# AaronZ345/StyleSinger

Hardware: AMD Instinct MI355X
Metric: mel-frames/sec (end-to-end infer incl. vocoder) (higher is better)
Workload: dtype f32; 1 GPU; c2: batch=8x8.0s utterances per GPU (T=1500 frames, Tp=28, Tr=1500), 100 mel + 2x100 f0 diffusion steps + HiFi-GAN-NSF, exact fp32 MFMA; global_batch=8, frames_per_utterance=1500, parallelism=dp1, diffusion_loops=hipGraph replay, hipgraph_captures=6, frame_bucket=64, mfma_precision=fp32, step_overlap=3 HIP streams: consecutive batches run concurrently

## Files before the change

include/stylesinger_hip.h:

```cpp
#ifndef STYLESINGER_HIP_H
#define STYLESINGER_HIP_H

#include <stdint.h>

#ifdef __cplusplus
extern "C" {
#endif

#define SS_ABI_VERSION 20
#define SS_MAX_TAPS 16
#define SS_MAX_LAYERS 32

const char* ss_last_error(void);
int ss_abi_version(void);
int ss_device_info(int dev, int* n_cu, char* arch, int arch_len);
int ss_struct_sizes(int64_t* out, int n);
int ss_set_tuning(const char* key, int value);
int ss_get_tuning(const char* key);
int ss_set_clock_probe(void* dev_u64x2);
int ss_set_q4_guard(void* dev_u32x2);
int ss_debug_null_launch(int grid, int block, void* stream);

enum {
  SS_EPI_STORE = 0,
// ... 14 lines not shown
  int32_t tap_off[SS_MAX_TAPS];
  const int32_t* lens;
  int32_t B, T;
  const float* a_bias;
  float a_scale;
  float a_lrelu;
  const float* W;
  int32_t N;
  int32_t Np;
  int32_t Kp;
  int32_t epi;
  const float* bias;
  float pre_scale;
  int32_t act;
  float act_slope;
  const float* E;
  int32_t lde;
  int64_t e_batch_stride;
  int32_t gate_mode;
  const float* R;
  int32_t ldr;
  int64_t r_batch_stride;
  float post_scale;
  int32_t accumulate;
  int32_t mask_rows;
  float* C;
  int32_t ldc;
  int64_t c_batch_stride;
  float* C2;
  int32_t ldc2;
  int64_t c2_batch_stride;
  int32_t Nh;
  float ddpm_recip, ddpm_recipm1, ddpm_c1, ddpm_c2, ddpm_sigma;
  const float* noise;
  uint64_t seed;
  const uint64_t* seed_dev;
  uint32_t step;
  int32_t tile;
  int32_t group_size;
  int64_t w_group_stride, bias_group_stride, a_bias_group_stride;
  int32_t mfma_bf16;
  int32_t ddpm_x0_pred;
  int32_t e_tiled;
  int32_t reserved2_;
} ss_conv_gemm_args;

int ss_conv_gemm(const ss_conv_gemm_args* args, void* stream);

int ss_gemm16_res(const ss_conv_gemm_args* args, int mt, void* stream);
int ss_gemm16_pick(int B, int T, int N);
int ss_gemm16_store(const ss_conv_gemm_args* args, int mt, void* stream);
int ss_gemm16_store_splitk(const ss_conv_gemm_args* args, int mt, int ksplit, float* partials, void* stream);
int ss_gemm16_ksplit_pick(int B, int T, int N, int K);

int ss_gemm16_resw(const ss_conv_gemm_args* args, const float* W16, int mt, void* stream);
int ss_pack_gemm16_weights(const float* src, float* dst, int Np, int Kp, void* stream);
int ss_wino43_gate16w(const ss_conv_gemm_args* args, const float* W16, int dilation, int mt, void* stream);
int ss_pack_gate16_weights(const float* src, float* dst, int Np, int Kp, void* stream);
int ss_wino43_gate16x(const ss_conv_gemm_args* args, const void* Wx, int dilation, int mt, void* stream);
int ss_split3_weights(const float* src, void* dst, int Np, int Kp, void* stream);
int ss_gemm16x_store(const ss_conv_gemm_args* args, const void* Wx, int mt, void* stream);
int ss_split3_gemm16_weights(const float* src, void* dst, int Np, int Kp, void* stream);
int64_t ss_split3_gemm16_elems(int Np, int Kp);
int ss_wino43_conv(const ss_conv_gemm_args* args, int k, int dilation, void* stream);
int ss_wino43_conv_ok(int C, int k, int dilation);
int ss_wino43_conv_ok4(int Cin, int Cout, int k, int dilation);
int ss_wino44_conv(const ss_conv_gemm_args* args, int k, int dilation, void* stream);
int ss_wino44_conv_ok(int C, int k, int dilation);
int ss_wino_gate(const ss_conv_gemm_args* args, int dilation, void* stream);
int ss_wino_weight_transform(const float* src, float* dst, int Cout, int Cin, void* stream);
int ss_wino43_gate(const ss_conv_gemm_args* args, int dilation, void* stream);
int ss_wino43_gate16(const ss_conv_gemm_args* args, int dilation, int mt, void* stream);
int ss_gate16_tile_addend(const float* E, int lde, int64_t e_batch_stride, float* E16, int B, int T, int Np, int dilation, int mt, void* stream);
int64_t ss_gate16_tiled_floats(int B, int T, int Np, int dilation, int mt);
int ss_wino43_gate16_pick(int B, int T, int Np, int dilation);
int ss_wino43_weight_transform(const float* src, float* dst, int Cout, int Cin, void* stream);

enum {
  SS_HEPI_STORE = 0,
  SS_HEPI_GATE = 1,
  SS_HEPI_RESX = 2
};
typedef struct ss_gemm_bf16_args {
  const uint16_t* A;
  int64_t a_batch_stride;
  int32_t lda;
  int32_t K;
  int32_t ntaps;
  int32_t tap_off[4];
  const int32_t* lens;
  int32_t B, T;
  const uint16_t* W;
  int64_t w_group_stride;
  int32_t N, Np;
  int32_t epi;
  int32_t act;
  const float* bias;
  int64_t bias_group_stride;
  const float* E;
  int32_t lde;
  int32_t gate_mode;
  int64_t e_batch_stride;
  float* X;
  int64_t x_batch_stride;
  int32_t ldx;
  float post_scale;
// ... 350 lines not shown
```

stylesinger_amd/csrc/common.h:

```cpp
#pragma once
#include <hip/hip_runtime.h>
#include <stdint.h>
#include <stdio.h>
#include <string.h>
#include <math.h>

#define SS_OK 0
#define SS_ERR_ARG (-1)
#define SS_ERR_HIP (-2)
#define SS_ERR_UNSUPPORTED (-3)

void ss_set_error(const char* fmt, ...);

#define SS_CHECK_ARG(cond, ...)            \
  do {                                     \
    if (!(cond)) {                         \
      ss_set_error(__VA_ARGS__);           \
      return SS_ERR_ARG;                   \
    }                                      \
  } while (0)

#define SS_CHECK_LAUNCH(name)                                                   \
  do {                                                                          \
    hipError_t e__ = hipGetLastError();                                         \
    if (e__ != hipSuccess) {                                                    \
      ss_set_error("%s: launch failed: %s", name, hipGetErrorString(e__));      \
      return SS_ERR_HIP;                                                        \
    }                                                                           \
  } while (0)

#define SS_PROPAGATE(expr)        \
  do {                            \
    int rc__ = (expr);            \
    if (rc__ != SS_OK) return rc__; \
  } while (0)

static inline int ss_cdiv(long a, long b) { return (int)((a + b - 1) / b); }

struct SsTuning { unsigned long long* clock_probe; int gate16; int gate256; int gate16_ks; int voc_wino_max_mb; int mel_tail; int gate128; int q4_force;
                  int layer512; int layer512_tail; int skip_dense; };
extern SsTuning g_ss_tuning;
extern unsigned int* g_ss_q4_guard;
struct ss_gemm_bf16_args;
int ss_q4_guard_launch(const ss_gemm_bf16_args* a, int which, void* stream);
int ss_n_cu();
struct ss_conv_gemm_args;
int ss_gemm16_store_partials(const ss_conv_gemm_args* args, int mt, int ksplit, float* partials, void* stream);

__device__ __forceinline__ int ss_uniform_len(const int* lens, int b, int T) {
  if (!lens) return T;
  const auto* p = reinterpret_cast<const __attribute__((address_space(4))) int*>(reinterpret_cast<uintptr_t>(lens));
  const int n = p[__builtin_amdgcn_readfirstlane(b)];
  return n < T ? (n < 0 ? 0 : n) : T;
}
__device__ __forceinline__ float ss_sigmoid(float x) { return 1.0f / (1.0f + expf(-x)); }
__device__ __forceinline__ float ss_sigmoid_fast(float x) { return __builtin_amdgcn_rcpf(1.0f + __expf(-x)); }
__device__ __forceinline__ float ss_tanh_fast(float x) { return 2.0f * __builtin_amdgcn_rcpf(1.0f + __expf(-2.0f * x)) - 1.0f; }
__device__ __forceinline__ float ss_gelu(float x) { return 0.5f * x * (1.0f + erff(x * 0.70710678118654752440f)); }
__device__ __forceinline__ float ss_mish(float x) {
  float sp = (x > 20.0f) ? x : log1pf(expf(x));
  return x * tanhf(sp);
}
__device__ __forceinline__ float ss_lrelu(float x, float slope) { return x >= 0.0f ? x : x * slope; }
__device__ __forceinline__ float ss_lrelu_max(float x, float sx) {
  float o;
  asm("v_max_f32 %0, %1, %2" : "=v"(o) : "v"(x), "v"(sx));
  return o;
}

enum SsAct { SS_ACT_NONE = 0, SS_ACT_RELU = 1, SS_ACT_GELU = 2, SS_ACT_MISH = 3, SS_ACT_TANH = 4, SS_ACT_LRELU = 5 };

__device__ __forceinline__ float ss_apply_act(float v, int act, float slope) {
  switch (act) {
    case SS_ACT_RELU: return fmaxf(v, 0.0f);
    case SS_ACT_GELU: return ss_gelu(v);
    case SS_ACT_MISH: return ss_mish(v);
    case SS_ACT_TANH: return tanhf(v);
    case SS_ACT_LRELU: return ss_lrelu(v, slope);
    default: return v;
  }
}

struct SsPhilox {
  uint32_t k0, k1;
  __device__ __forceinline__ SsPhilox(uint64_t seed) : k0((uint32_t)seed), k1((uint32_t)(seed >> 32)) {}
  __device__ __forceinline__ void round(uint32_t (&c)[4], uint32_t ka, uint32_t kb) const {
    const uint32_t M0 = 0xD2511F53u, M1 = 0xCD9E8D57u;
    uint32_t hi0 = __umulhi(M0, c[0]), lo0 = M0 * c[0];
    uint32_t hi1 = __umulhi(M1, c[2]), lo1 = M1 * c[2];
    uint32_t n0 = hi1 ^ c[1] ^ ka, n1 = lo1, n2 = hi0 ^ c[3] ^ kb, n3 = lo0;
    c[0] = n0; c[1] = n1; c[2] = n2; c[3] = n3;
  }
  __device__ __forceinline__ void gen(uint32_t c0, uint32_t c1, uint32_t c2, uint32_t c3, uint32_t (&out)[4]) const {
    uint32_t c[4] = {c0, c1, c2, c3};
    uint32_t ka = k0, kb = k1;
#pragma unroll
    for (int i = 0; i < 10; ++i) {
      round(c, ka, kb);
      ka += 0x9E3779B9u;
      kb += 0xBB67AE85u;
// ... 52 lines not shown
```

stylesinger_amd/csrc/diffusion.hip:

```cpp
#include "common.h"
#include <stdlib.h>
#include <cmath>
#include <vector>
#include "../../include/stylesinger_hip.h"

namespace {

inline int64_t align_up(int64_t x, int64_t a) { return (x + a - 1) / a * a; }
inline int round_up32(int x) { return (x + 31) / 32 * 32; }
constexpr int MTR = 2;

enum StackKind {
  STACK_FP32,
  STACK_PAIR16,
  STACK_FUSED16,
};
enum GateEntry { GATE_CONV, GATE_WINO23, GATE_WINO43, GATE_WINO43_16, GATE_WINO43_16W, GATE_WINO43_16X };
enum ProjEntry { PROJ_CONV, PROJ_RES16, PROJ_RES16W };
enum SkipEntry { SKIP_CONV, SKIP_STORE16, SKIP_SPLITK, SKIP_X3 };
struct LayerForm {
  int d;
  GateEntry gate;
  int mt;
  int64_t e16_floats;
// ... 179 lines not shown
  a.lda = ld;
  a.a_batch_stride = (int64_t)T * ld;
}
template <class Args, class P> inline void set_c(Args& a, P* p, int ld, int T) {
  a.C = p;
  a.ldc = ld;
  a.c_batch_stride = (int64_t)T * ld;
}
template <class Args> inline void set_taps3(Args& a, int d) {
  a.ntaps = 3;
  a.tap_off[0] = -d;
  a.tap_off[1] = 0;
  a.tap_off[2] = d;
}
inline void set_groups(ss_conv_gemm_args& a, const ss_wavenet* net, int B, int64_t gs_w, int64_t gs_bias, int64_t gs_a_bias = 0) {
  if (net->n_groups <= 1) return;
  a.group_size = B / net->n_groups;
  a.w_group_stride = gs_w;
  a.bias_group_stride = gs_bias;
  a.a_bias_group_stride = gs_a_bias;
}

int precompute_cond(const ss_wavenet* net, const StackForm& sf, const float* cond, const int32_t* lens, int B, int T, const WsLayout& w, hipStream_t stream) {
  const int NE = net->L * 2 * net->C;
  if (sf.cond16) {
    SS_PROPAGATE(ss_to_bf16(cond, nullptr, w.condh, B, T, net->cond_dim, net->cond_dim, net->cond_dim, nullptr, 0, 0, stream));
    ss_gemm_bf16_args h = base_args_h(net, B, T, lens);
    set_a(h, w.condh, net->cond_dim, T);
    h.K = net->cond_dim;
    h.W = net->w_cond_h;
    h.w_group_stride = net->gs_w_cond_h;
    h.N = NE;
    h.Np = NE;
    h.epi = SS_HEPI_STORE;
    h.bias = net->b_cond;
    h.bias_group_stride = net->gs_b_cond;
    set_c(h, w.E, NE, T);
    h.mask_rows = 0;
    return ss_gemm_bf16(&h, stream);
  }
  ss_conv_gemm_args a = base_args(B, T, lens);
  set_a(a, cond, net->cond_dim, T);
  a.Cin = net->cond_dim;
  a.W = net->w_cond;
  a.N = NE;
  a.Np = NE;
  a.Kp = round_up32(net->cond_dim);
  a.epi = SS_EPI_STORE;
  a.bias = net->b_cond;
  set_c(a, w.E, NE, T);
  a.mask_rows = 0;
  a.mfma_bf16 = sf.outer_bf16;
  set_groups(a, net, B, net->gs_w_cond, net->gs_b_cond);
  SS_PROPAGATE(ss_conv_gemm(&a, stream));
  for (int l = 0; l < net->L; ++l) {
    const float* El = w.E + (int64_t)l * 2 * net->C;
    if (w.E512)
      SS_PROPAGATE(ss_layer512_tile_addend(El, NE, (int64_t)T * NE, w.E512 + (int64_t)l * w.e512_layer, B, T, stream));
    if (w.E512h)
      SS_PROPAGATE(ss_layer512_tile_addend_f16(El, NE, (int64_t)T * NE, w.E512h + (int64_t)l * w.e512h_layer, sf.n_esets, w.e512h_set, B, T, stream));
    if (w.E16[l])
      SS_PROPAGATE(ss_gate16_tile_addend(El, NE, (int64_t)T * NE, w.E16[l], B, T, 2 * net->C, sf.layer[l].d, sf.layer[l].mt, stream));
  }
  return SS_OK;
}

int skip_gemm_f32(const ss_wavenet* net, const StackForm& sf, const int32_t* lens, int B, int T, const WsLayout& w, hipStream_t stream, bool leave_partials) {
  const int C = net->C, L = net->L;
  ss_conv_gemm_args k = base_args(B, T, lens);
  set_a(k, w.GA, L * C, T);
  k.Cin = L * C;
  k.W = net->w_skipall;
  k.N = C;
  k.Np = round_up32(C);
  k.Kp = L * C;
  k.epi = SS_EPI_STORE;
  k.bias = net->b_skipall;
  set_c(k, sf.skip_folded ? w.G : w.S, C, T);
  if (sf.skip_folded) k.act = SS_ACT_RELU;
  k.tile = SS_TILE_64x64;
  k.mfma_bf16 = sf.conv_bf16;
  set_groups(k, net, B, net->gs_w_skipall, net->gs_b_skipall);
  switch (sf.skip) {
    case SKIP_X3:
      k.w_group_stride = net->gs_w_skipall_x3;
      return ss_gemm16x_store(&k, net->w_skipall_x3, sf.mt16, stream);
    case SKIP_SPLITK:
      return leave_partials && sf.partials_ok ? ss_gemm16_store_partials(&k, 4, sf.ksplit, w.KP, stream) : ss_gemm16_store_splitk(&k, 4, sf.ksplit, w.KP, stream);
    case SKIP_STORE16: return ss_gemm16_store(&k, sf.mt16, stream);
    default: return ss_conv_gemm(&k, stream);
  }
}

int run_stack_f32(const ss_wavenet* net, const StackForm& sf, int step, const int32_t* lens, int B, int T, const WsLayout& w, hipStream_t stream, bool leave_partials) {
  const int C = net->C, L = net->L;
  const int NE = L * 2 * C;
  const int ldg = sf.defer ? L * C : C;
  for (int l = 0; l < L; ++l) {
    const LayerForm& y = sf.layer[l];
    ss_conv_gemm_args a = base_args(B, T, lens);
    set_a(a, w.X, C, T);
    a.Cin = C;
    set_taps3(a, y.d);
    a.a_bias = net->dstep + ((int64_t)step * L + l) * C;
    a.W = net->w_dil[l];
    a.N = C;
    a.Np = 2 * C;
// ... 453 lines not shown
  const float fa = (f0_a[i] + 1.0f) / 2.0f * (10.0f - 6.0f) + 6.0f;
  const float fb = (f0_b[i] + 1.0f) / 2.0f * (10.0f - 6.0f) + 6.0f;
  const float f = fb / 2.0f + fa / 2.0f;
  const float u = ub / 2.0f + ua / 2.0f;
  pitch_pred[(int64_t)i * 2 + 0] = f;
  pitch_pred[(int64_t)i * 2 + 1] = u;
  float hz = exp2f(f);
  if (u > 0.0f) hz = 0.0f;
  if (mel2ph[i] == 0) hz = 0.0f;
  f0_denorm[i] = hz;
  coarse[i] = f0_to_coarse(hz);
}

__global__ void pitch_given_kernel(const float* __restrict__ f0_log2, const float* __restrict__ uv, const int64_t* __restrict__ mel2ph,
                                   float* __restrict__ pitch_pred, float* __restrict__ f0_denorm, int64_t* __restrict__ coarse, int n) {
  const int i = blockIdx.x * blockDim.x + threadIdx.x;
  if (i >= n) return;
  const float f = f0_log2[i] / 2.0f + f0_log2[i] / 2.0f;
  const float u = uv[i] / 2.0f + uv[i] / 2.0f;
  pitch_pred[(int64_t)i * 2 + 0] = f;
  pitch_pred[(int64_t)i * 2 + 1] = u;
  float hz = exp2f(f);
  if (u > 0.0f) hz = 0.0f;
  if (mel2ph[i] == 0) hz = 0.0f;
  f0_denorm[i] = hz;
  coarse[i] = f0_to_coarse(hz);
}

inline int grid_for(int64_t n) {
  int64_t g = (n + 255) / 256;
  return (int)(g < 1 ? 1 : (g > 8192 ? 8192 : g));
}

}

extern "C" int64_t ss_wavenet_workspace_bytes(const ss_wavenet* net, int B, int T) {
  if (!net || B <= 0 || T <= 0) return -1;
  return ws_layout(net, resolve_form(net, B, T), B, T, nullptr).bytes;
}

static int mel_input_proj(const ss_wavenet* net, const float* x_in, const int32_t* lens, int B, int T, const WsLayout& w, hipStream_t stream) {
  const int C = net->C, M = net->in_dim;
  ss_conv_gemm_args a = base_args(B, T, lens);
  set_a(a, x_in, M, T);
  a.Cin = M;
  a.W = net->w_in;
  a.N = C;
  a.Np = round_up32(C);
  a.Kp = round_up32(M);
  a.epi = SS_EPI_STORE;
  a.bias = net->b_in;
  a.act = SS_ACT_RELU;
  set_c(a, w.X, C, T);
  return ss_conv_gemm(&a, stream);
}

__global__ __launch_bounds__(256) void mel_tail_kernel(const SkipSrc src, const float* __restrict__ Wf, const float* __restrict__ bf,
                                                       float* __restrict__ x, const float* __restrict__ noise, uint64_t seed,
                                                       const uint64_t* __restrict__ seed_dev, uint32_t step, float recip, float recipm1, float c1,
                                                       float c2, float sigma, const float* __restrict__ Win, const float* __restrict__ bin,
                                                       float* __restrict__ X, const int32_t* __restrict__ lens, int B, int T, int C, int M, int Kp_in) {
  extern __shared__ __attribute__((aligned(16))) float smem_mt[];
  float* gs = smem_mt;
  float* xs = smem_mt + MTR * C;
  const int64_t n_rows = (int64_t)B * T, r0 = (int64_t)blockIdx.x * MTR;
  const int tid = threadIdx.x, C4 = C / 4;
  for (int idx = tid; idx < MTR * C4; idx += 256) {
    const int row = idx / C4, q = idx - row * C4;
    float4 v = make_float4(0.f, 0.f, 0.f, 0.f);
    if (r0 + row < n_rows) {
      const int64_t i = r0 + row;
      v = skip_load4(src, src.bias, i, C, 4 * q, lens && (int)(i % T) >= lens[i / T]);
    }
    *reinterpret_cast<float4*>(gs + row * C + 4 * q) = v;
  }
  for (int idx = tid; idx < MTR * Kp_in; idx += 256) xs[idx] = 0.f;
  __syncthreads();
  const SsPhilox rng(seed + (seed_dev ? seed_dev[0] : 0ull));
  for (int idx = tid; idx < MTR * M; idx += 256) {
    const int row = idx / M, n = idx - row * M;
    const int64_t i = r0 + row;
    if (i >= n_rows) continue;
    const float* wr = Wf + (int64_t)n * C;
    const float* gr = gs + row * C;
    float acc = 0.f;
#pragma unroll 8
    for (int q = 0; q < C4; ++q) {
      const float4 wv = *reinterpret_cast<const float4*>(wr + 4 * q), gv = *reinterpret_cast<const float4*>(gr + 4 * q);
      acc = fmaf(gv.w, wv.w, fmaf(gv.z, wv.z, fmaf(gv.y, wv.y, fmaf(gv.x, wv.x, acc))));
    }
    const float eps = acc + bf[n];
    const int b = (int)(i / T), t = (int)(i % T);
    const float xv = x[i * M + n];
    float z = 0.f;
    if (sigma != 0.f) {
      if (noise) z = noise[i * M + n];
      else {
        float z4[4];
        ss_mel_draw4(rng, (uint32_t)(t >> 2), (uint32_t)M, (uint32_t)n, (uint32_t)b, step, z4);
        z = z4[t & 3];
      }
    }
    float xn = ss_ddpm_update(xv, eps, recip, recipm1, c1, c2, sigma, z, 0);
    if (lens && t >= lens[b]) xn = 0.f;
    x[i * M + n] = xn;
    xs[row * Kp_in + n] = xn;
  }
// ... 412 lines not shown
```

stylesinger_amd/csrc/gemm16.hip:

```cpp
#include "common.h"
#include "device_prims.h"
#include "../../include/stylesinger_hip.h"
#include <type_traits>

namespace {

using namespace ss_dev;

constexpr int BK = 32;
constexpr int LD = BK;
constexpr int BN = 64;
constexpr int NBUF = 3;

template <int MT, int KCH, bool WL>
__device__ __forceinline__ void gemm16_res_body(const ss_conv_gemm_args& a, const float* __restrict__ W16, int m_tiles_per_item, int m_tiles, int n_tiles,
                                                const int block_id, float* __restrict__ lds_) {
  constexpr int BM = 16 * MT;
  constexpr int GROUPS = BM / 8;
  constexpr int DPW = (GROUPS + 3) / 4;
  static_assert(GROUPS % 4 == 0, "row groups must split evenly over the 4 waves");
  float* const As0 = static_cast<float*>(__builtin_assume_aligned(lds_, 16));
  float* const As1 = As0 + BM * LD;
  float* const As2 = As1 + BM * LD;

// ... 233 lines not shown
#pragma unroll
      for (int m = 0; m < MT; ++m) acc[m] = __builtin_amdgcn_mfma_f32_16x16x4f32(af[m][h].x, bf[h].x, acc[m], 0, 0, 0);
      __builtin_amdgcn_sched_barrier(0);
#pragma unroll
      for (int m = 0; m < MT; ++m) acc[m] = __builtin_amdgcn_mfma_f32_16x16x4f32(af[m][h].y, bf[h].y, acc[m], 0, 0, 0);
      __builtin_amdgcn_sched_barrier(0);
#pragma unroll
      for (int m = 0; m < MT; ++m) acc[m] = __builtin_amdgcn_mfma_f32_16x16x4f32(af[m][h].z, bf[h].z, acc[m], 0, 0, 0);
      __builtin_amdgcn_sched_barrier(0);
#pragma unroll
      for (int m = 0; m < MT; ++m) acc[m] = __builtin_amdgcn_mfma_f32_16x16x4f32(af[m][h].w, bf[h].w, acc[m], 0, 0, 0);
      __builtin_amdgcn_sched_barrier(0);
    }
  };
  dma(A0, B0, kbeg);
  int c = kbeg;
  for (; c + 2 <= kchunks; c += 2) {
    chunk(A0, B0, A1, B1, c, true);
    chunk(A1, B1, A0, B0, c + 1, c + 2 < kchunks);
  }
  if (c < kchunks) chunk(A0, B0, A1, B1, c, false);

  const int col = n0 + 16 * wave + lc;
  const bool col_ok = col < a.N;
  const int oob = col_ok ? 0 : (int)0x80000000;
  if (ksplit > 1) {
    const __amdgpu_buffer_rsrc_t rsrc_p = __builtin_amdgcn_make_buffer_rsrc(
        uniform_ptr(P + ((int64_t)ksi * a.B + b) * a.T * a.N), 0, __builtin_amdgcn_readfirstlane((int)((int64_t)a.T * a.N * 4)), 0x00020000);
    const int p_base = ((t0 + 4 * kg) * a.N + col) * 4 + oob;
#pragma unroll
    for (int m = 0; m < MT; ++m)
#pragma unroll
      for (int r = 0; r < 4; ++r) {
        const float v = acc[m][r];
        __builtin_amdgcn_raw_buffer_store_b32(__builtin_bit_cast(unsigned, v), rsrc_p, p_base, (16 * m + r) * a.N * 4, 0);
      }
    return;
  }
  const float bs = (a.bias && col_ok) ? a.bias[(int64_t)grp_w * a.bias_group_stride + col] : 0.f;
  const int row_lim = a.mask_rows ? (len < a.T ? len : a.T) : a.T;
  const int c_base = ((t0 + 4 * kg) * a.ldc + col) * 4 + oob;
  const bool relu = a.act == SS_ACT_RELU;
#pragma unroll
  for (int m = 0; m < MT; ++m)
#pragma unroll
    for (int r = 0; r < 4; ++r) {
      float o = acc[m][r] + bs;
      if (relu) o = fmaxf(o, 0.f);
      if (t0 + 16 * m + 4 * kg + r >= row_lim) o = 0.f;
      __builtin_amdgcn_raw_buffer_store_b32(__builtin_bit_cast(unsigned, o), rsrc_c, c_base, (16 * m + r) * a.ldc * 4, 0);
    }
}

__global__ void splitk_reduce_kernel(const float* __restrict__ P, const ss_conv_gemm_args a, int ksplit) {
  const int64_t per = (int64_t)a.B * a.T * a.N;
  const int n4 = a.N / 4;
  for (int64_t i = blockIdx.x * (int64_t)blockDim.x + threadIdx.x; i < per / 4; i += (int64_t)gridDim.x * blockDim.x) {
    const int c4 = (int)(i % n4) * 4;
    const int64_t r = i / n4;
    const int b = (int)(r / a.T), t = (int)(r % a.T);
    float4 v = *reinterpret_cast<const float4*>(P + i * 4);
    for (int s = 1; s < ksplit; ++s) {
      const float4 u = *reinterpret_cast<const float4*>(P + s * per + i * 4);
      v.x += u.x; v.y += u.y; v.z += u.z; v.w += u.w;
    }
    if (a.bias) {
      const float* bp = a.bias + (a.group_size > 0 ? (int64_t)(b / a.group_size) * a.bias_group_stride : 0) + c4;
      v.x += bp[0]; v.y += bp[1]; v.z += bp[2]; v.w += bp[3];
    }
    if (a.act == SS_ACT_RELU) v = make_float4(fmaxf(v.x, 0.f), fmaxf(v.y, 0.f), fmaxf(v.z, 0.f), fmaxf(v.w, 0.f));
    if (a.mask_rows && a.lens && t >= a.lens[b]) v = make_float4(0.f, 0.f, 0.f, 0.f);
    *reinterpret_cast<float4*>(a.C + (int64_t)b * a.c_batch_stride + (int64_t)t * a.ldc + c4) = v;
  }
}

template <int MT>
int launch_store(const ss_conv_gemm_args& a, int ksplit, float* P, hipStream_t stream, bool reduce = true) {
  constexpr int BM = 16 * MT;
  const int m_tiles_per_item = ss_cdiv(a.T, BM);
  const int m_tiles = m_tiles_per_item * a.B;
  const int n_tiles = ss_cdiv(a.N, BN);
  const int grid = ss_cdiv(m_tiles, 8) * 8 * n_tiles;
  hipLaunchKernelGGL(gemm16_store_kernel<MT>, dim3(grid * ksplit), dim3(256), 0, stream, a, m_tiles_per_item, m_tiles, n_tiles, ksplit, P);
  if (ksplit > 1 && reduce) {
    const int64_t n = (int64_t)a.B * a.T * a.N / 4;
    hipLaunchKernelGGL(splitk_reduce_kernel, dim3((int)((n + 255) / 256 < 2048 ? (n + 255) / 256 : 2048)), dim3(256), 0, stream, P, a, ksplit);
  }
  return 0;
}

template <int MT, int KCH>
int launch_res(const ss_conv_gemm_args& a, const float* W16, hipStream_t stream) {
  constexpr int BM = 16 * MT;
  const int m_tiles_per_item = ss_cdiv(a.T, BM);
  const int m_tiles = m_tiles_per_item * a.B;
  const int n_tiles = ss_cdiv(a.N, BN);
  const int grid = ss_cdiv(m_tiles, 8) * 8 * n_tiles;
  if (W16) hipLaunchKernelGGL((gemm16_res_kernel<MT, KCH, true>), dim3(grid), dim3(256), 0, stream, a, W16, m_tiles_per_item, m_tiles, n_tiles);
  else hipLaunchKernelGGL((gemm16_res_kernel<MT, KCH, false>), dim3(grid), dim3(256), 0, stream, a, W16, m_tiles_per_item, m_tiles, n_tiles);
  return 0;
}

__global__ void pack_gemm16_kernel(const float* __restrict__ src, float* __restrict__ dst, int Np, int Kp) {
  const int64_t n = (int64_t)Np * Kp;
  const int kch = Kp / BK;
  for (int64_t i = blockIdx.x * (int64_t)blockDim.x + threadIdx.x; i < n; i += (int64_t)gridDim.x * blockDim.x) {
    const int kk = (int)(i % Kp), col = (int)(i / Kp);
    const int nt = col / BN, w = (col % BN) / 16, lc = col % 16;
    const int j = kk / BK, kg = (kk % BK) / 8, h = (kk % 8) / 4, e = kk % 4;
    dst[((((int64_t)(nt * 4 + w) * kch + j) * 2 + h) * 64 + kg * 16 + lc) * 4 + e] = src[i];
  }
}

}

extern "C" int ss_gemm16_pick(int B, int T, int N) {
  const int n_tiles = ss_cdiv(N, BN);
  int best = 4;
  long best_cost = -1;
  const bool tiny = (long)ss_cdiv(T, 64) * B * n_tiles * 2 <= ss_n_cu();
  for (int mt = 8; mt >= (tiny ? 2 : 4); mt -= 2) {
    const long wgs = (long)ss_cdiv(T, 16 * mt) * B * n_tiles;
    const long cost = (long)mt * ss_cdiv(wgs, ss_n_cu());
    if (best_cost < 0 || cost < best_cost) {
      best_cost = cost;
      best = mt;
    }
  }
  return best;
}

static int gemm16_res_impl(const ss_conv_gemm_args* args, const float* W16, int mt, void* stream, const char* who) {
  SS_CHECK_ARG(args != nullptr, "%s: null args", who);
  const ss_conv_gemm_args& a = *args;
  SS_CHECK_ARG(a.A && a.W && a.C && a.R, "%s: null A/W/C/R", who);
  SS_CHECK_ARG(a.ntaps == 1 && a.tap_off[0] == 0, "%s: one tap at offset 0 only", who);
  SS_CHECK_ARG(a.Kp == a.Cin && (a.Kp == 192 || a.Kp == 256) && (a.lda & 3) == 0, "%s: K=%d must be 192 or 256 (= Kp), lda %% 4 == 0", who, a.Cin);
  SS_CHECK_ARG(a.N > 0 && a.N <= a.Np && (a.Np & 15) == 0, "%s: bad N=%d Np=%d", who, a.N, a.Np);
  SS_CHECK_ARG(!W16 || (a.N % BN) == 0, "%s: the fetch-order weights need N %% 64 == 0 (N=%d)", who, a.N);
  SS_CHECK_ARG(a.a_scale == 1.0f && a.a_lrelu == 1.0f && a.a_bias == nullptr && a.mfma_bf16 == 0, "%s: no A prologue, fp32 only", who);
// ... 18 lines not shown
extern "C" int ss_gemm16_resw(const ss_conv_gemm_args* args, const float* W16, int mt, void* stream) {
  SS_CHECK_ARG(W16 != nullptr, "ss_gemm16_resw: null W16");
  return gemm16_res_impl(args, W16, mt, stream, "ss_gemm16_resw");
}

extern "C" int ss_pack_gemm16_weights(const float* src, float* dst, int Np, int Kp, void* stream) {
  SS_CHECK_ARG(src && dst && src != dst && Np > 0 && (Np % BN) == 0 && Kp > 0 && (Kp % BK) == 0, "ss_pack_gemm16_weights: Np %% 64, Kp %% 32, out of place");
  const int64_t n = (int64_t)Np * Kp;
  const int grid = (int)((n + 255) / 256 < 4096 ? (n + 255) / 256 : 4096);
  hipLaunchKernelGGL(pack_gemm16_kernel, dim3(grid), dim3(256), 0, (hipStream_t)stream, src, dst, Np, Kp);
  SS_CHECK_LAUNCH("ss_pack_gemm16_weights");
  return SS_OK;
}

static int gemm16_store_impl(const ss_conv_gemm_args* args, int mt, int ksplit, float* partials, void* stream, const char* who, bool reduce = true) {
  SS_CHECK_ARG(args != nullptr, "%s: null args", who);
  const ss_conv_gemm_args& a = *args;
  SS_CHECK_ARG(a.A && a.W && a.C, "%s: null A/W/C", who);
  SS_CHECK_ARG(a.ntaps == 1 && a.tap_off[0] == 0, "%s: one tap at offset 0 only", who);
  SS_CHECK_ARG(a.Kp == a.Cin && (a.Kp % BK) == 0 && (a.lda & 3) == 0, "%s: K=%d must equal Kp and be a multiple of 32, lda %% 4 == 0", who, a.Cin);
  SS_CHECK_ARG(a.N > 0 && a.N <= a.Np, "%s: bad N=%d Np=%d", who, a.N, a.Np);
  SS_CHECK_ARG(a.a_scale == 1.0f && a.a_lrelu == 1.0f && a.a_bias == nullptr && a.mfma_bf16 == 0 && a.pre_scale == 1.0f && a.post_scale == 1.0f &&
                   a.R == nullptr && !a.accumulate && (a.act == SS_ACT_NONE || a.act == SS_ACT_RELU),
               "%s: plain C = act(A.W^T + bias) only (act none | relu), fp32", who);
  SS_CHECK_ARG((int64_t)a.T * a.lda * 4 < (1ll << 31) && (int64_t)a.T * a.ldc * 4 < (1ll << 31) && (int64_t)a.Np * a.Kp * 4 < (1ll << 31),
               "%s: item too large for 32-bit offsets", who);
  SS_CHECK_ARG(mt == 0 || mt == 4 || mt == 6 || mt == 8, "%s: mt=%d must be 0 (auto), 4, 6 or 8", who, mt);
  SS_CHECK_ARG(ksplit >= 1 && ksplit <= 16 && ksplit <= a.Kp / BK && (ksplit == 1 || (partials && (a.N & 3) == 0 && (a.ldc & 3) == 0)),
               "%s: ksplit=%d needs a partials buffer of ksplit*B*T*N floats, N %% 4 == 0 and at most Kp/32 slices", who, ksplit);
  if (mt == 0) mt = ksplit > 1 ? 4 : ss_gemm16_pick(a.B, a.T, a.N);
  if (mt == 2) mt = 4;
  hipStream_t s = (hipStream_t)stream;
  switch (mt) {
    case 4: launch_store<4>(a, ksplit, partials, s, reduce); break;
    case 6: launch_store<6>(a, ksplit, partials, s, reduce); break;
    default: launch_store<8>(a, ksplit, partials, s, reduce); break;
  }
  SS_CHECK_LAUNCH(who);
  return SS_OK;
}

extern "C" int ss_gemm16_store(const ss_conv_gemm_args* args, int mt, void* stream) {
  return gemm16_store_impl(args, mt, 1, nullptr, stream, "ss_gemm16_store");
}

extern "C" int ss_gemm16_store_splitk(const ss_conv_gemm_args* args, int mt, int ksplit, float* partials, void* stream) {
  return gemm16_store_impl(args, mt, ksplit, partials, stream, "ss_gemm16_store_splitk");
}

int ss_gemm16_store_partials(const ss_conv_gemm_args* args, int mt, int ksplit, float* partials, void* stream) {
  return gemm16_store_impl(args, mt, ksplit, partials, stream, "ss_gemm16_store_partials", false);
}

extern "C" int ss_gemm16_ksplit_pick(int B, int T, int N, int K) {
  const long wgs = (long)ss_cdiv(T, 64) * B * ss_cdiv(N, BN);
  const int n_cu = ss_n_cu();
  if (wgs * 2 > n_cu || K < 512) return 1;
  int s = (int)(n_cu / wgs);
  const int smax = K / BK / 8;
  if (s > smax) s = smax;
  if (s > 16) s = 16;
  return s < 1 ? 1 : s;
}
```

stylesinger_amd/csrc/hifigan.hip:

```cpp
#include "common.h"
#include "../../include/stylesinger_hip.h"

namespace {

constexpr int NH = 9;
constexpr int HOP_MAX = 1024;
constexpr size_t LDS_MAX = 160 * 1024;

inline int64_t align_up(int64_t x, int64_t a) { return (x + a - 1) / a * a; }
inline int round_up32(int x) { return (x + 31) / 32 * 32; }

struct HgWs {
  int32_t* lens;
  double* base;
  double* q;
  float* r0;
  float* har;
  float* pre;
  float* x;
  float* xs;
  float* ta;
  float* tb;
  int64_t bytes;
};
// ... 394 lines not shown

  {
    ss_conv_gemm_args a = base_args(B, T, w.lens);
    a.A = mel;
    a.lda = 80;
    a.a_batch_stride = (int64_t)T * 80;
    a.Cin = 80;
    a.ntaps = 7;
    for (int j = 0; j < 7; ++j) a.tap_off[j] = j - 3;
    a.W = hg->w_pre;
    a.N = hg->c0;
    a.Np = round_up32(hg->c0);
    a.Kp = 96;
    a.epi = SS_EPI_STORE;
    a.bias = hg->b_pre;
    a.C = w.pre;
    a.ldc = hg->c0;
    a.c_batch_stride = (int64_t)T * hg->c0;
    a.mfma_bf16 = hg->mfma_bf16;
    SS_PROPAGATE(ss_conv_gemm(&a, stream));
  }

  const float* cur = w.pre;
  int rows_in = T, cin = hg->c0, R = 1;
  for (int i = 0; i < hg->n_ups; ++i) {
    const int u = hg->up_rate[i], ku = hg->up_k[i];
    const int cout = hg->c0 >> (i + 1);
    const int pad = (ku - u) / 2;
    const int nph0 = u - pad;
    const int rows_out = rows_in * u;
    const int32_t* lens_in = w.lens + (int64_t)i * B;
    const int32_t* lens_out = w.lens + (int64_t)(i + 1) * B;
    for (int g = 0; g < 2; ++g) {
      const int nph = g == 0 ? nph0 : u - nph0;
      ss_conv_gemm_args a = base_args(B, rows_in, lens_in);
      a.A = cur;
      a.lda = cin;
      a.a_batch_stride = (int64_t)rows_in * cin;
      a.Cin = cin;
      a.ntaps = 2;
      a.tap_off[0] = g == 0 ? 0 : 1;
      a.tap_off[1] = g == 0 ? -1 : 0;
      a.a_lrelu = 0.1f;
      a.W = hg->w_up[i][g];
      a.N = nph * cout;
      a.Np = round_up32(nph * cout);
      a.Kp = round_up32(cin);
      a.epi = SS_EPI_STORE;
      a.bias = hg->b_up[i];
      a.C = w.x + (g == 0 ? 0 : (int64_t)nph0 * cout);
      a.ldc = u * cout;
      a.c_batch_stride = (int64_t)rows_in * u * cout;
      a.mfma_bf16 = hg->mfma_bf16;
      SS_PROPAGATE(ss_conv_gemm(&a, stream));
    }
    R *= u;
    {
      int s = 1;
      for (int j = i + 1; j < hg->n_ups; ++j) s *= hg->up_rate[j];
      const int kk = (i + 1 < hg->n_ups) ? 2 * s : 1;
      const int pd = (i + 1 < hg->n_ups) ? s / 2 : 0;
      const int npos = 64;
      int nchunk = 1;
      auto lds_of = [&](int cc) { return ((size_t)kk * cc + (size_t)npos * s + kk) * sizeof(float); };
      while (lds_of(ss_cdiv(cout, nchunk)) > LDS_MAX && nchunk < cout) nchunk *= 2;
      const int cc = ss_cdiv(cout, nchunk);
      const size_t lds = lds_of(cc);
      SS_CHECK_ARG(lds <= LDS_MAX, "ss_hifigan_forward: noise conv of stage %d needs %zu bytes of LDS", i, lds);
      const int tiles = (rows_out + npos - 1) / npos;
      hipLaunchKernelGGL(noise_conv_kernel, dim3(B * tiles, ss_cdiv(cout, cc)), dim3(256), lds, stream, har, hg->w_noise[i], hg->b_noise[i],
                         w.x, lens_out, w.lens + (int64_t)hg->n_ups * B, B, rows_out, L, cout, cc, kk, s, pd, npos);
      SS_CHECK_LAUNCH("noise_conv_kernel");
    }
    const float inv = 1.0f / (float)hg->n_kernels;
    for (int j = 0; j < hg->n_kernels; ++j) {
      const int k = hg->rb_k[j];
      const float* xin = w.x;
      for (int m = 0; m < 3; ++m) {
        const int d = hg->rb_d[j][m];
        const bool wino = hg->wino && !hg->mfma_bf16;
        const float* ww1 = wino && ss_wino43_conv_ok(cout, k, d) ? hg->w_rb1_wino[i][j][m] : nullptr;
        const float* ww2 = wino && ss_wino43_conv_ok(cout, k, 1) ? hg->w_rb2_wino[i][j][m] : nullptr;
        SS_PROPAGATE(conv_same(xin, B, rows_out, cout, lens_out, hg->w_rb1[i][j][m], ww1, hg->b_rb1[i][j][m], k, d, 0.1f, 1, nullptr, 1.0f,
                               0, w.ta, hg->mfma_bf16, stream));
        if (m < 2) {
          SS_PROPAGATE(conv_same(w.ta, B, rows_out, cout, lens_out, hg->w_rb2[i][j][m], ww2, hg->b_rb2[i][j][m], k, 1, 1.0f, 0, xin, 1.0f,
                                 0, w.tb, hg->mfma_bf16, stream));
          xin = w.tb;
        } else {
          SS_PROPAGATE(conv_same(w.ta, B, rows_out, cout, lens_out, hg->w_rb2[i][j][m], ww2, hg->b_rb2[i][j][m], k, 1, 1.0f, 0, xin, inv,
                                 j > 0, w.xs, hg->mfma_bf16, stream));
        }
      }
    }
    cur = w.xs;
    rows_in = rows_out;
    cin = cout;
  }
  {
    const int k = 7;
    const size_t lds = ((size_t)(256 + k - 1) * (cin + 1) + (size_t)k * cin) * sizeof(float);
    SS_CHECK_ARG(lds <= LDS_MAX, "ss_hifigan_forward: conv_post over %d channels needs %zu bytes of LDS", cin, lds);
    const int tiles = (int)((L + 255) / 256);
    hipLaunchKernelGGL(conv_post_kernel, dim3(B * tiles), dim3(256), lds, stream, cur, hg->w_post, hg->b_post, wav,
                       w.lens + (int64_t)hg->n_ups * B, B, L, cin, k);
    SS_CHECK_LAUNCH("conv_post_kernel");
  }
// ... 3 lines not shown
```

stylesinger_amd/lib.py:

```python
import ctypes as C
import os

import torch

from . import abi
from .abi import declarations, declared_symbols

HERE = os.path.dirname(os.path.abspath(__file__))
LIB_PATH = os.environ.get("SS_LIB_PATH") or os.path.join(HERE, "libstylesinger_hip.so")

SS_MAX_TAPS, SS_MAX_LAYERS, SS_HG_MAX_UPS, SS_HG_MAX_KERNELS = (abi.DEFINES[n] for n in ("SS_MAX_TAPS", "SS_MAX_LAYERS", "SS_HG_MAX_UPS", "SS_HG_MAX_KERNELS"))
ABI_VERSION = abi.DEFINES["SS_ABI_VERSION"]
ALIGN_MAX_T, ALIGN_MAX_LC = abi.DEFINES["SS_ALIGN_MAX_T"], abi.DEFINES["SS_ALIGN_MAX_LC"]
EPI_STORE, EPI_GATE, EPI_RESSKIP, EPI_DDPM = (abi.ENUMS["SS_EPI_" + n] for n in ("STORE", "GATE", "RESSKIP", "DDPM"))
ACT_NONE, ACT_RELU, ACT_GELU, ACT_MISH, ACT_TANH, ACT_LRELU = (abi.ENUMS[f"SS_ACT_{n}_"] for n in ("NONE", "RELU", "GELU", "MISH", "TANH", "LRELU"))
HEPI_STORE, HEPI_GATE, HEPI_RESX = (abi.ENUMS["SS_HEPI_" + n] for n in ("STORE", "GATE", "RESX"))

_STRUCT_SIZES_ORDER = ("ss_conv_gemm_args", "ss_wavenet", "ss_hifigan", "ss_gemm_bf16_args", "ss_f0track_params", "ss_layer512_args")
ConvGemmArgs, WaveNet, HifiGan, GemmBf16Args, F0TrackParams, Layer512Args = (abi.STRUCTURES[n] for n in _STRUCT_SIZES_ORDER)


class StyleSingerHipError(RuntimeError):
    pass

# ... 95 lines not shown
def gate16_tile_addend(E, *, B, T, Np, lde, e_bs, dilation, mt):
    n = load().ss_gate16_tiled_floats(B, T, Np, int(dilation), int(mt))
    out = torch.empty(n, device=E.device, dtype=torch.float32)
    check(load().ss_gate16_tile_addend(ptr(E), lde, e_bs, ptr(out), B, T, Np, int(dilation), int(mt), stream_ptr()), "ss_gate16_tile_addend")
    return out


def wino_gate(A, Wt, out, *, dilation, **kw):
    kw.setdefault("epi", EPI_GATE)
    a = _fill_args(A, Wt, out, **kw)
    check(load().ss_wino_gate(C.byref(a), int(dilation), stream_ptr()), "ss_wino_gate")


def wino43_gate(A, Wt, out, *, dilation, **kw):
    kw.setdefault("epi", EPI_GATE)
    a = _fill_args(A, Wt, out, **kw)
    check(load().ss_wino43_gate(C.byref(a), int(dilation), stream_ptr()), "ss_wino43_gate")


def pack_gemm16_weights(Wp, Kp):
    Wp = Wp.contiguous().float()
    out = torch.empty_like(Wp)
    check(load().ss_pack_gemm16_weights(ptr(Wp), ptr(out), Wp.shape[0], Kp, stream_ptr()), "ss_pack_gemm16_weights")
    return out


def pack_gate16_weights(Wp, Kp):
    Wp = Wp.contiguous().float()
    out = torch.empty_like(Wp)
    check(load().ss_pack_gate16_weights(ptr(Wp), ptr(out), Wp.shape[0], Kp, stream_ptr()), "ss_pack_gate16_weights")
    return out


def wino43_gate16(A, Wt, out, *, dilation, mt=0, W16=None, **kw):
    kw.setdefault("epi", EPI_GATE)
    a = _fill_args(A, Wt, out, **kw)
    if W16 is not None:
        check(load().ss_wino43_gate16w(C.byref(a), ptr(W16), int(dilation), int(mt), stream_ptr()), "ss_wino43_gate16w")
        return
    check(load().ss_wino43_gate16(C.byref(a), int(dilation), int(mt), stream_ptr()), "ss_wino43_gate16")


def gemm16_res(A, W, out, *, mt=0, W16=None, **kw):
    a = _fill_args(A, W, out, **kw)
    if W16 is not None:
        check(load().ss_gemm16_resw(C.byref(a), ptr(W16), int(mt), stream_ptr()), "ss_gemm16_resw")
        return
    check(load().ss_gemm16_res(C.byref(a), int(mt), stream_ptr()), "ss_gemm16_res")


def gemm16_store(A, W, out, *, mt=0, **kw):
    a = _fill_args(A, W, out, **kw)
    check(load().ss_gemm16_store(C.byref(a), int(mt), stream_ptr()), "ss_gemm16_store")


def gemm16_store_splitk(A, W, out, *, ksplit, mt=0, **kw):
    a = _fill_args(A, W, out, **kw)
    part = torch.empty(max(1, ksplit) * a.B * a.T * a.N, device=out.device, dtype=torch.float32)
    check(load().ss_gemm16_store_splitk(C.byref(a), int(mt), int(ksplit), ptr(part), stream_ptr()), "ss_gemm16_store_splitk")


def wino43_weight(w):
    w = w.contiguous().float()
    out = torch.empty(w.shape[0], w.shape[1], 6, device=w.device, dtype=torch.float32)
    check(load().ss_wino43_weight_transform(ptr(w), ptr(out), w.shape[0], w.shape[1], stream_ptr()), "ss_wino43_weight_transform")
    return out


def wino43_group_weight(w):
    w = w.contiguous().float()
    Cout, Cin, k = w.shape
    G = (k + 2) // 3
    wp = torch.zeros(Cout, Cin, 3 * G, device=w.device, dtype=torch.float32)
    wp[..., :k] = w
    return torch.cat([wino43_weight(wp[..., 3 * g:3 * g + 3]) for g in range(G)], dim=-1).contiguous()


def wino43_conv(A, W, out, *, k, dilation, **kw):
    taps = [(j - (k - 1) // 2) * dilation for j in range(k)]
    a = _fill_args(A, W, out, taps=taps, **kw)
    check(load().ss_wino43_conv(C.byref(a), k, dilation, stream_ptr()), "ss_wino43_conv")
    return out


WINO44_G = (
    (-1 / 2, 0.0, 0.0, 0.0),
    (-1 / 3, -1 / 3, -1 / 3, -1 / 3),
    (1 / 9, -1 / 9, 1 / 9, -1 / 9),
    (1 / 36, 1 / 18, 1 / 9, 2 / 9),
    (-1 / 60, 1 / 30, -1 / 15, 2 / 15),
    (32 / 45, 16 / 45, 8 / 45, 4 / 45),
    (0.0, 0.0, 0.0, 1.0),
)


def wino44_conv_ok(C, k, dilation):
    return int(load().ss_wino44_conv_ok(int(C), int(k), int(dilation)))


def wino44_group_weight(w):
    Cout, Cin, k = w.shape
    G = (k + 3) // 4
    wp = torch.zeros(Cout, Cin, G, 4, device=w.device, dtype=torch.float64)
    wp.view(Cout, Cin, 4 * G)[..., :k] = w.double()
    g = torch.tensor(WINO44_G, device=w.device, dtype=torch.float64)
    return torch.einsum("jt,oigt->oigj", g, wp).reshape(Cout, Cin, 7 * G).float().contiguous()
# ... 364 lines not shown
```

Before: 45320 mel-frames/s.

## Add multi-tap fp32 MFMA GEMM kernel for conv layers with fused input leaky-ReLU

Adds a new gemm16 taps kernel that treats a 1-3 tap convolution as one GEMM. It loops over the taps and K-chunks with double-buffered LDS DMA, applies leaky-ReLU to the A tile in LDS, and fuses bias and ReLU into the store. The kernel is routed in through a dispatcher for the diffusion cond/input projections and the HiFi-GAN upsample convs with N>=64, replacing the generic conv_gemm path when its constraints hold. The aim is to cut the overhead of the generic conv kernel and of a separate activation pass. The cost is another specialised code path with its own tile-size heuristics that could underperform on some shapes.

```diff
diff --git a/include/stylesinger_hip.h b/include/stylesinger_hip.h
--- a/include/stylesinger_hip.h
+++ b/include/stylesinger_hip.h
@@ -90,6 +90,8 @@
 int ss_gemm16_store(const ss_conv_gemm_args* args, int mt, void* stream);
 int ss_gemm16_store_splitk(const ss_conv_gemm_args* args, int mt, int ksplit, float* partials, void* stream);
 int ss_gemm16_ksplit_pick(int B, int T, int N, int K);
+int ss_gemm16_store_taps(const ss_conv_gemm_args* args, int mt, void* stream);
+int ss_gemm16_store_taps_ok(const ss_conv_gemm_args* args);
 
 int ss_gemm16_resw(const ss_conv_gemm_args* args, const float* W16, int mt, void* stream);
 int ss_pack_gemm16_weights(const float* src, float* dst, int Np, int Kp, void* stream);
diff --git a/stylesinger_amd/csrc/common.h b/stylesinger_amd/csrc/common.h
--- a/stylesinger_amd/csrc/common.h
+++ b/stylesinger_amd/csrc/common.h
@@ -46,6 +46,7 @@
 int ss_n_cu();
 struct ss_conv_gemm_args;
 int ss_gemm16_store_partials(const ss_conv_gemm_args* args, int mt, int ksplit, float* partials, void* stream);
+int ss_conv_gemm_or_taps(const ss_conv_gemm_args* args, void* stream);
 
 __device__ __forceinline__ int ss_uniform_len(const int* lens, int b, int T) {
   if (!lens) return T;
diff --git a/stylesinger_amd/csrc/diffusion.hip b/stylesinger_amd/csrc/diffusion.hip
--- a/stylesinger_amd/csrc/diffusion.hip
+++ b/stylesinger_amd/csrc/diffusion.hip
@@ -255,7 +255,7 @@
   a.mask_rows = 0;
   a.mfma_bf16 = sf.outer_bf16;
   set_groups(a, net, B, net->gs_w_cond, net->gs_b_cond);
-  SS_PROPAGATE(ss_conv_gemm(&a, stream));
+  SS_PROPAGATE(ss_conv_gemm_or_taps(&a, stream));
   for (int l = 0; l < net->L; ++l) {
     const float* El = w.E + (int64_t)l * 2 * net->C;
     if (w.E512)
@@ -815,7 +815,7 @@
   a.bias = net->b_in;
   a.act = SS_ACT_RELU;
   set_c(a, w.X, C, T);
-  return ss_conv_gemm(&a, stream);
+  return ss_conv_gemm_or_taps(&a, stream);
 }
 
 __global__ __launch_bounds__(256) void mel_tail_kernel(const SkipSrc src, const float* __restrict__ Wf, const float* __restrict__ bf,
diff --git a/stylesinger_amd/csrc/gemm16.hip b/stylesinger_amd/csrc/gemm16.hip
--- a/stylesinger_amd/csrc/gemm16.hip
+++ b/stylesinger_amd/csrc/gemm16.hip
@@ -309,6 +309,151 @@
     }
 }
 
+template <int MT, bool LRELU>
+__global__ __launch_bounds__(256, 3) void gemm16_taps_kernel(const ss_conv_gemm_args a, int m_tiles_per_item, int m_tiles, int n_tiles) {
+  constexpr int BM = 16 * MT;
+  constexpr int GROUPS = BM / 8;
+  constexpr int DPW = GROUPS / 4;
+  static_assert(GROUPS % 4 == 0, "row groups must split evenly over the 4 waves");
+  __shared__ __attribute__((aligned(16))) float A0[BM * LD];
+  __shared__ __attribute__((aligned(16))) float A1[BM * LD];
+  __shared__ __attribute__((aligned(16))) float B0[4 * 16 * LD];
+  __shared__ __attribute__((aligned(16))) float B1[4 * 16 * LD];
+
+  const int id = blockIdx.x;
+  const int grp = id / (8 * n_tiles);
+  const int rem = id % (8 * n_tiles);
+  const int mt = grp * 8 + (rem & 7);
+  const int nt = rem >> 3;
+  if (mt >= m_tiles) return;
+  const int b = mt / m_tiles_per_item;
+  const int t0 = (mt % m_tiles_per_item) * BM;
+  const int n0 = nt * BN;
+  const int tid = threadIdx.x, lane = tid & 63, wave = tid >> 6;
+  const int lc = lane & 15, kg = lane >> 4;
+  const int len = ss_uniform_len(a.lens, b, a.T);
+  const int grp_w = a.group_size > 0 ? b / a.group_size : 0;
+  const int kch = a.Kp / BK;
+  const int nchunks = a.ntaps * kch;
+  const int ldw = a.ntaps * a.Kp;
+
+  const __amdgpu_buffer_rsrc_t rsrc_a = __builtin_amdgcn_make_buffer_rsrc(
+      uniform_ptr(a.A + (int64_t)b * a.a_batch_stride), 0, __builtin_amdgcn_readfirstlane(len * a.lda * 4), 0x00020000);
+  const __amdgpu_buffer_rsrc_t rsrc_w = __builtin_amdgcn_make_buffer_rsrc(
+      uniform_ptr(a.W + (int64_t)grp_w * a.w_group_stride), 0, __builtin_amdgcn_readfirstlane(a.Np * ldw * 4), 0x00020000);
+  const __amdgpu_buffer_rsrc_t rsrc_c = __builtin_amdgcn_make_buffer_rsrc(
+      uniform_ptr(a.C + (int64_t)b * a.c_batch_stride), 0, __builtin_amdgcn_readfirstlane((int)((int64_t)a.T * a.ldc * 4)), 0x00020000);
+
+  int a_voff[DPW], b_voff[2];
+#pragma unroll
+  for (int j = 0; j < DPW; ++j) {
+    const int row = 8 * (wave + 4 * j) + (lane >> 3);
+    a_voff[j] = ((t0 + row) * a.lda + (((lane & 7) ^ swz16(row)) << 2)) * 4;
+  }
+#pragma unroll
+  for (int j = 0; j < 2; ++j) {
+    const int row = 8 * j + (lane >> 3);
+    b_voff[j] = ((n0 + 16 * wave + row) * ldw + (((lane & 7) ^ swz16(row)) << 2)) * 4;
+  }
+  const int sh0 = a.tap_off[0] * a.lda * 4, sh1 = a.ntaps > 1 ? a.tap_off[1] * a.lda * 4 : 0, sh2 = a.ntaps > 2 ? a.tap_off[2] * a.lda * 4 : 0;
+  auto dma = [&](float* Abuf, float* Bbuf, int c, int ao) {
+#pragma unroll
+    for (int j = 0; j < DPW; ++j) glds16(rsrc_a, Abuf + (wave + 4 * j) * 8 * LD, a_voff[j] + ao, 0);
+    const int so = c * (BK * 4);
+#pragma unroll
+    for (int j = 0; j < 2; ++j) glds16(rsrc_w, Bbuf + (wave * 16 + 8 * j) * LD, b_voff[j], so);
+  };
+  const int rd0 = lc * LD + (((2 * kg) ^ swz16(lc)) << 2), rd1 = lc * LD + (((2 * kg + 1) ^ swz16(lc)) << 2);
+  const float slope = a.a_lrelu;
+
+  f32x4 acc[MT];
+#pragma unroll
+  for (int m = 0; m < MT; ++m)
+#pragma unroll
+    for (int r = 0; r < 4; ++r) acc[m][r] = 0.f;
+
+  auto chunk = [&](float* Ac, const float* Bc, float* An, float* Bn, int c, bool more, int ao_next) {
+    wait_vmcnt<0>();
+    if constexpr (LRELU) {
+      __builtin_amdgcn_sched_barrier(0);
+      float4 v[DPW];
+#pragma unroll
+      for (int j = 0; j < DPW; ++j) v[j] = *reinterpret_cast<const float4*>(Ac + (wave + 4 * j) * 8 * LD + lane * 4);
+#pragma unroll
+      for (int j = 0; j < DPW; ++j) {
+        v[j].x = ss_lrelu_max(v[j].x, slope * v[j].x); v[j].y = ss_lrelu_max(v[j].y, slope * v[j].y);
+        v[j].z = ss_lrelu_max(v[j].z, slope * v[j].z); v[j].w = ss_lrelu_max(v[j].w, slope * v[j].w);
+        *reinterpret_cast<float4*>(Ac + (wave + 4 * j) * 8 * LD + lane * 4) = v[j];
+      }
+      __builtin_amdgcn_s_waitcnt(0xc07f);
+      __builtin_amdgcn_sched_barrier(0);
+    }
+    __builtin_amdgcn_s_barrier();
+    float4 af[MT][2], bf[2];
+#pragma unroll
+    for (int m = 0; m < MT; ++m) {
+      af[m][0] = *reinterpret_cast<const float4*>(Ac + 16 * m * LD + rd0);
+      af[m][1] = *reinterpret_cast<const float4*>(Ac + 16 * m * LD + rd1);
+    }
+    bf[0] = *reinterpret_cast<const float4*>(Bc + wave * 16 * LD + rd0);
+    bf[1] = *reinterpret_cast<const float4*>(Bc + wave * 16 * LD + rd1);
+    __builtin_amdgcn_sched_barrier(0);
+    if (more) dma(An, Bn, c + 1, ao_next);
+    __builtin_amdgcn_sched_barrier(0);
+#pragma unroll
+    for (int h = 0; h < 2; ++h) {
+#pragma unroll
+      for (int m = 0; m < MT; ++m) acc[m] = __builtin_amdgcn_mfma_f32_16x16x4f32(af[m][h].x, bf[h].x, acc[m], 0, 0, 0);
+      __builtin_amdgcn_sched_barrier(0);
+#pragma unroll
+      for (int m = 0; m < MT; ++m) acc[m] = __builtin_amdgcn_mfma_f32_16x16x4f32(af[m][h].y, bf[h].y, acc[m], 0, 0, 0);
+      __builtin_amdgcn_sched_barrier(0);
+#pragma unroll
+      for (int m = 0; m < MT; ++m) acc[m] = __builtin_amdgcn_mfma_f32_16x16x4f32(af[m][h].z, bf[h].z, acc[m], 0, 0, 0);
+      __builtin_amdgcn_sched_barrier(0);
+#pragma unroll
+      for (int m = 0; m < MT; ++m) acc[m] = __builtin_amdgcn_mfma_f32_16x16x4f32(af[m][h].w, bf[h].w, acc[m], 0, 0, 0);
+      __builtin_amdgcn_sched_barrier(0);
+    }
+  };
+  dma(A0, B0, 0, sh0);
+  int tap = 0, kc = 0, ao = 0;
+#define SS_TAPS_ADVANCE()                                           \
+  do {                                                              \
+    if (++kc == kch) {                                              \
+      kc = 0;                                                       \
+      ++tap;                                                        \
+    }                                                               \
+    ao = (tap == 0 ? sh0 : (tap == 1 ? sh1 : sh2)) + kc * (BK * 4); \
+  } while (0)
+  int c = 0;
+  for (; c + 2 <= nchunks; c += 2) {
+    SS_TAPS_ADVANCE();
+    chunk(A0, B0, A1, B1, c, true, ao);
+    SS_TAPS_ADVANCE();
+    chunk(A1, B1, A0, B0, c + 1, c + 2 < nchunks, ao);
+  }
+  if (c < nchunks) chunk(A0, B0, A1, B1, c, false, 0);
+#undef SS_TAPS_ADVANCE
+
+  const int col = n0 + 16 * wave + lc;
+  const bool col_ok = col < a.N;
+  const int oob = col_ok ? 0 : (int)0x80000000;
+  const float bs = (a.bias && col_ok) ? a.bias[(int64_t)grp_w * a.bias_group_stride + col] : 0.f;
+  const int row_lim = a.mask_rows ? (len < a.T ? len : a.T) : a.T;
+  const int c_base = ((t0 + 4 * kg) * a.ldc + col) * 4 + oob;
+  const bool relu = a.act == SS_ACT_RELU;
+#pragma unroll
+  for (int m = 0; m < MT; ++m)
+#pragma unroll
+    for (int r = 0; r < 4; ++r) {
+      float o = acc[m][r] + bs;
+      if (relu) o = fmaxf(o, 0.f);
+      if (t0 + 16 * m + 4 * kg + r >= row_lim) o = 0.f;
+      __builtin_amdgcn_raw_buffer_store_b32(__builtin_bit_cast(unsigned, o), rsrc_c, c_base, (16 * m + r) * a.ldc * 4, 0);
+    }
+}
+
 __global__ void splitk_reduce_kernel(const float* __restrict__ P, const ss_conv_gemm_args a, int ksplit) {
   const int64_t per = (int64_t)a.B * a.T * a.N;
   const int n4 = a.N / 4;
@@ -343,6 +488,18 @@
     const int64_t n = (int64_t)a.B * a.T * a.N / 4;
     hipLaunchKernelGGL(splitk_reduce_kernel, dim3((int)((n + 255) / 256 < 2048 ? (n + 255) / 256 : 2048)), dim3(256), 0, stream, P, a, ksplit);
   }
+  return 0;
+}
+
+template <int MT>
+int launch_taps(const ss_conv_gemm_args& a, hipStream_t stream) {
+  constexpr int BM = 16 * MT;
+  const int m_tiles_per_item = ss_cdiv(a.T, BM);
+  const int m_tiles = m_tiles_per_item * a.B;
+  const int n_tiles = ss_cdiv(a.N, BN);
+  const int grid = ss_cdiv(m_tiles, 8) * 8 * n_tiles;
+  if (a.a_lrelu != 1.0f) hipLaunchKernelGGL((gemm16_taps_kernel<MT, true>), dim3(grid), dim3(256), 0, stream, a, m_tiles_per_item, m_tiles, n_tiles);
+  else hipLaunchKernelGGL((gemm16_taps_kernel<MT, false>), dim3(grid), dim3(256), 0, stream, a, m_tiles_per_item, m_tiles, n_tiles);
   return 0;
 }
 
@@ -467,6 +624,57 @@
   return gemm16_store_impl(args, mt, ksplit, partials, stream, "ss_gemm16_store_partials", false);
 }
 
+extern "C" int ss_gemm16_store_taps_ok(const ss_conv_gemm_args* args) {
+  if (!args) return 0;
+  const ss_conv_gemm_args& a = *args;
+  if (a.epi != SS_EPI_STORE || a.mfma_bf16 || a.accumulate || a.R || a.a_bias) return 0;
+  if (a.a_scale != 1.0f || a.pre_scale != 1.0f || a.post_scale != 1.0f) return 0;
+  if (!(a.a_lrelu == 1.0f || (a.a_lrelu > 0.0f && a.a_lrelu < 1.0f))) return 0;
+  if (a.act != SS_ACT_NONE && a.act != SS_ACT_RELU) return 0;
+  if (a.ntaps < 1 || a.ntaps > 3) return 0;
+  if (a.Kp <= 0 || (a.Kp % BK) != 0 || a.Cin <= 0 || (a.Cin & 3) != 0 || a.Cin > a.Kp || a.Kp - a.Cin >= BK) return 0;
+  if ((a.lda & 3) != 0 || a.lda < a.Cin) return 0;
+  if (a.N <= 0 || a.N > a.Np || a.ldc < a.N) return 0;
+  if ((int64_t)a.Np * a.ntaps * a.Kp * 4 >= (1ll << 31)) return 0;
+  return 1;
+}
+
+static bool gemm16_taps_fits(const ss_conv_gemm_args& a) {
+  int64_t tmax = 0;
+  for (int j = 0; j < a.ntaps; ++j) tmax = tmax > llabs((long long)a.tap_off[j]) ? tmax : llabs((long long)a.tap_off[j]);
+  return ((int64_t)a.T + 256 + tmax) * a.lda * 4 < (1ll << 31) && ((int64_t)a.T + 256) * a.ldc * 4 < (1ll << 31);
+}
+
+extern "C" int ss_gemm16_store_taps(const ss_conv_gemm_args* args, int mt, void* stream) {
+  const char* who = "ss_gemm16_store_taps";
+  SS_CHECK_ARG(args != nullptr, "%s: null args", who);
+  const ss_conv_gemm_args& a = *args;
+  SS_CHECK_ARG(a.A && a.W && a.C && a.B > 0 && a.T > 0, "%s: null A/W/C or empty launch", who);
+  SS_CHECK_ARG(ss_gemm16_store_taps_ok(args),
+               "%s: plain C = act(sum_taps lrelu(A).W^T + bias) only: <= 3 taps, fp32, act none | relu, no R / accumulate / a_bias / scales, "
+               "Kp - Cin < 32, lda %% 4 == 0 (ntaps=%d Cin=%d Kp=%d lda=%d)", who, a.ntaps, a.Cin, a.Kp, a.lda);
+  SS_CHECK_ARG(gemm16_taps_fits(a), "%s: item too large for 32-bit offsets", who);
+  SS_CHECK_ARG(mt == 0 || mt == 4 || mt == 6 || mt == 8, "%s: mt=%d must be 0 (auto), 4, 6 or 8", who, mt);
+  if (mt == 0) {
+    const long wgs8 = (long)ss_cdiv(a.T, 128) * a.B * ss_cdiv(a.N, BN);
+    mt = wgs8 >= 6l * ss_n_cu() ? (a.a_lrelu != 1.0f ? 4 : 8) : ss_gemm16_pick(a.B, a.T, a.N);
+    if (mt == 2) mt = 4;
+  }
+  hipStream_t s = (hipStream_t)stream;
+  switch (mt) {
+    case 4: launch_taps<4>(a, s); break;
+    case 6: launch_taps<6>(a, s); break;
+    default: launch_taps<8>(a, s); break;
+  }
+  SS_CHECK_LAUNCH(who);
+  return SS_OK;
+}
+
+int ss_conv_gemm_or_taps(const ss_conv_gemm_args* args, void* stream) {
+  if (ss_gemm16_store_taps_ok(args) && gemm16_taps_fits(*args)) return ss_gemm16_store_taps(args, 0, stream);
+  return ss_conv_gemm(args, stream);
+}
+
 extern "C" int ss_gemm16_ksplit_pick(int B, int T, int N, int K) {
   const long wgs = (long)ss_cdiv(T, 64) * B * ss_cdiv(N, BN);
   const int n_cu = ss_n_cu();
diff --git a/stylesinger_amd/csrc/hifigan.hip b/stylesinger_amd/csrc/hifigan.hip
--- a/stylesinger_amd/csrc/hifigan.hip
+++ b/stylesinger_amd/csrc/hifigan.hip
@@ -470,7 +470,8 @@
       a.ldc = u * cout;
       a.c_batch_stride = (int64_t)rows_in * u * cout;
       a.mfma_bf16 = hg->mfma_bf16;
-      SS_PROPAGATE(ss_conv_gemm(&a, stream));
+      if (a.N >= 64) SS_PROPAGATE(ss_conv_gemm_or_taps(&a, stream));
+      else SS_PROPAGATE(ss_conv_gemm(&a, stream));
     }
     R *= u;
     {
diff --git a/stylesinger_amd/lib.py b/stylesinger_amd/lib.py
--- a/stylesinger_amd/lib.py
+++ b/stylesinger_amd/lib.py
@@ -171,6 +171,16 @@
 def gemm16_store(A, W, out, *, mt=0, **kw):
     a = _fill_args(A, W, out, **kw)
     check(load().ss_gemm16_store(C.byref(a), int(mt), stream_ptr()), "ss_gemm16_store")
+
+
+def gemm16_store_taps_ok(**kw):
+    a = _fill_args(None, None, None, **kw)
+    return int(load().ss_gemm16_store_taps_ok(C.byref(a)))
+
+
+def gemm16_store_taps(A, W, out, *, mt=0, **kw):
+    a = _fill_args(A, W, out, **kw)
+    check(load().ss_gemm16_store_taps(C.byref(a), int(mt), stream_ptr()), "ss_gemm16_store_taps")
 
 
 def gemm16_store_splitk(A, W, out, *, ksplit, mt=0, **kw):
```

Result: no change. 45500 mel-frames/s, median of 6 (+0.4%).
